# sarpel/wakeword_trainer_home

Hardware: AMD Instinct MI355X
Metric: training samples/sec (16kHz x 1.5s clips) (higher is better)
Workload: dtype bf16; 1 GPU; BASELINE config 2: cnn_small + log-mel(40) + SpecAugment, fwd/bwd + clip + AdamW, 16 kHz x 1.5 s clips resident in HBM; batch_per_gpu=512, activation_storage=bf16, arithmetic=f32, global_batch=512, n_samples=24000, parallelism=single, ranks_seen=1, hip_graph=False

## Files before the change

### include/wwhip.h

```cpp
#ifndef WWHIP_H
#define WWHIP_H

#include <stddef.h>
#include <stdint.h>

#ifdef __cplusplus
extern "C" {
#endif

#define WW_ABI_VERSION 15

#define WW_OK 0
#define WW_E_INVALID (-1)
#define WW_E_HIP (-2)
#define WW_E_WORKSPACE (-3)
#define WW_E_UNSUPPORTED (-4)

typedef struct ww_ctx ww_ctx;
typedef void *ww_stream_t;

int ww_abi_version(void);
const char *ww_last_error(void);
int ww_ctx_create(int device, ww_ctx **out);
int ww_ctx_destroy(ww_ctx *ctx);

typedef struct {
    uint64_t step;
    float lr;
    int32_t parity;
    float loss_scale;
    int32_t growth_tracker;
    int32_t reserved[2];
} ww_step_ctl;
int ww_ctx_bind_step_ctl(ww_ctx *ctx, const ww_step_ctl *ctl_dev );
int ww_step_ctl_advance(ww_ctx *ctx, ww_stream_t stream);

typedef struct {
    int32_t sample_rate;
    int32_t n_fft;
    int32_t hop;
    int32_t n_mels;
    int32_t n_mfcc;
    float f_min;
// ... 44 lines not shown
                     uint64_t sample_offset, int32_t *choice_out, void *scratch, size_t scratch_bytes,
                     ww_stream_t stream);

typedef struct {
    const float *gamma;
    const float *beta;
    float *running_mean;
    float *running_var;
    float momentum;
    float eps;
    int32_t training;
} ww_bn_t;

#define WW_C 64
#define WW_ACT_F32 0
#define WW_ACT_BF16 1
#define WW_ACT_F16 2
#define WW_MAX_PARTIALS 1024
size_t ww_layer_scratch_bytes(void);

int ww_conv_stem_fwd(ww_ctx *ctx, int act_dtype, const float *x, const float *w, int B, int Hin, int Win, void *y,
                     const ww_bn_t *bn, float *ss_out, float *mr_out, void *scratch, ww_stream_t stream);
int ww_dwconv3x3_fwd(ww_ctx *ctx, int act_dtype, const void *y_in, const float *ss_in, const float *w, int B, int H,
                     int W, void *y, const ww_bn_t *bn, float *ss_out, float *mr_out, void *scratch,
                     ww_stream_t stream);
int ww_pwconv1x1_fwd(ww_ctx *ctx, int act_dtype, const void *y_in, const float *ss_in, const float *w, int B, int H,
                     int W, void *y, const ww_bn_t *bn, float *ss_out, float *mr_out, void *scratch,
                     ww_stream_t stream);
int ww_gap_fwd(ww_ctx *ctx, int act_dtype, const void *y, const float *ss, const float *mr, int B, int H, int W,
               float *pool, ww_stream_t stream);
int ww_head_fwd(ww_ctx *ctx, const float *pool, int B, int HW, const float *fc_w, const float *fc_b,
                float dropout_p, int training, uint64_t seed, uint64_t step, uint64_t sample_offset, float *pd,
                float *logits, ww_stream_t stream);

int ww_head_bwd(ww_ctx *ctx, const float *dlogits, const float *pd, const float *pool, int B, int HW,
                const float *fc_w, float dropout_p, int training, uint64_t seed, uint64_t step,
                uint64_t sample_offset, const float *gamma_last, const float *mr_last, float *dfc_w,
                float *dfc_b, float *dpool, float *coef_last, float *dgamma_last, float *dbeta_last,
                ww_stream_t stream);
int ww_pwconv1x1_bwd(ww_ctx *ctx, int act_dtype, const void *g, const float *dpool, const void *y_out,
                     const float *ss_out, const float *coef, const void *y_in, const float *ss_in, const float *mr_in,
                     const float *gamma_in, const float *w, int B, int H, int W, void *g_in, float *dw,
                     float *coef_in, float *dgamma_in, float *dbeta_in, void *scratch, ww_stream_t stream);
int ww_dwconv3x3_bwd(ww_ctx *ctx, int act_dtype, const void *g, const void *y_out, const float *coef, const void *y_in,
                     const float *ss_in, const float *mr_in, const float *gamma_in, const float *w, int B,
                     int H, int W, void *g_in, float *dw, float *coef_in, float *dgamma_in,
                     float *dbeta_in, void *scratch, ww_stream_t stream);
int ww_conv_stem_bwd(ww_ctx *ctx, int act_dtype, const void *g, const void *y_out, const float *coef, const float *x,
                     int B, int Hin, int Win, float *dw, void *scratch, ww_stream_t stream);

#define WW_CNN_SMALL_NPTR 47
size_t ww_cnn_small_workspace_bytes(int B, int F, int T, int act_dtype);
int ww_cnn_small_fwd(ww_ctx *ctx, int act_dtype, void *const *params, const float *x, int B, int F, int T, int training,
                     float bn_momentum, float bn_eps, float dropout_p, uint64_t seed, uint64_t step,
                     uint64_t sample_offset, void *ws, size_t ws_bytes, float *logits, ww_stream_t stream);
#define WW_BWD_ALL 0
#define WW_BWD_LATE 1
#define WW_BWD_EARLY 2
int ww_cnn_small_bwd(ww_ctx *ctx, int act_dtype, void *const *params, void *const *grads, const float *x, const float *dlogits,
                     int B, int F, int T, float dropout_p, uint64_t seed, uint64_t step, uint64_t sample_offset,
                     void *ws, size_t ws_bytes, int part, ww_stream_t stream);

#define WW_LOSS_CE 0
#define WW_LOSS_FOCAL 1
typedef struct {
    float loss;
// ... 155 lines not shown
```

### wakeword_trainer_home_amd/_native.py

```python
import contextlib
import ctypes as C
import math
import os
from pathlib import Path

import torch

_LIB_PATH = Path(__file__).resolve().parent / "csrc" / "libwwhip.so"
_lib = None
_ctx = {}

ABI_VERSION = 15
BWD_ALL, BWD_LATE, BWD_EARLY = 0, 1, 2
ACT_F32, ACT_BF16, ACT_F16 = 0, 1, 2
LOSS_CE, LOSS_FOCAL = 0, 1
WAVE_F32, WAVE_I16 = 0, 1
CNN_SMALL_NPTR = 47


class NativeError(RuntimeError):
    pass


class FeatCfg(C.Structure):
    _fields_ = [("sample_rate", C.c_int32), ("n_fft", C.c_int32), ("hop", C.c_int32), ("n_mels", C.c_int32),
                ("n_mfcc", C.c_int32), ("f_min", C.c_float), ("f_max", C.c_float), ("log_eps", C.c_float)]


class SpecAugCfg(C.Structure):
    _fields_ = [("freq_mask_param", C.c_int32), ("time_mask_param", C.c_int32), ("n_freq_masks", C.c_int32),
                ("n_time_masks", C.c_int32), ("freq_mask_prob", C.c_float), ("time_mask_prob", C.c_float)]


class BN(C.Structure):
    _fields_ = [("gamma", C.c_void_p), ("beta", C.c_void_p), ("running_mean", C.c_void_p),
                ("running_var", C.c_void_p), ("momentum", C.c_float), ("eps", C.c_float), ("training", C.c_int32)]


class AudioAugCfg(C.Structure):
    _fields_ = [("rir_prob", C.c_float), ("noise_prob", C.c_float), ("snr_min_db", C.c_float), ("snr_max_db", C.c_float)]


class LinearEpi(C.Structure):
    _fields_ = [("act", C.c_int32), ("dropout_p", C.c_float), ("seed", C.c_uint64), ("step", C.c_uint64),
                ("sample_offset", C.c_uint64)]
# ... 89 lines not shown
    "ww_dwconv_nhwc_fwd": (C.c_int, [_vp, _vp, _vp, _i, _i, _i, _i, _i, _i, _vp, _vp]),
    "ww_dwconv_nhwc_bwd": (C.c_int, [_vp, _vp, _vp, _vp, _i, _i, _i, _i, _i, _i, _vp, _vp, _vp, _vp]),
    "ww_pool_hw_fwd": (C.c_int, [_vp, _vp, _i, _i, _i, _vp, _vp]),
    "ww_scale_bc_fwd": (C.c_int, [_vp, _vp, _vp, _i, _i, _i, _vp, _vp]),
    "ww_scale_bc_bwd_gate": (C.c_int, [_vp, _vp, _vp, _i, _i, _i, _vp, _vp]),
    "ww_scale_pool_bwd": (C.c_int, [_vp, _vp, _vp, _vp, _i, _i, _i, _vp, _vp]),
    "ww_se_bwd_scratch_bytes": (_sz, [_i, _i, _i]),
    "ww_se_fwd": (C.c_int, [_vp, _vp, _i, _i, _i, _i] + [_vp] * 9),
    "ww_se_bwd": (C.c_int, [_vp] * 8 + [_i, _i, _i, _i] + [_vp] * 6 + [_sz, _vp]),
    "ww_stem3x3s2_bn_act_fwd": (C.c_int, [_vp, _vp, _vp, _i, _i, _i, _i, C.POINTER(BN), _i, _vp, _vp, _vp, _vp, _vp, _vp]),
    "ww_stem3x3s2_bwd_dw": (C.c_int, [_vp, _vp, _vp, _i, _i, _i, _i, _vp, _vp, _vp]),
    "ww_im2col3x3s2": (C.c_int, [_vp, _vp, _i, _i, _i, _vp, _vp]),
    "ww_add_f32": (C.c_int, [_vp, _vp, _vp, _sz, _vp, _vp]),
    "ww_gru_workspace_bytes": (_sz, [_i, _i, _i, _i]),
    "ww_gru_fwd": (C.c_int, [_vp, _i, _vp, C.c_long, _vp, _vp, _vp, _vp, _vp, _i, _i, _i, _i, _i, _vp, C.c_long, _vp, _vp, _sz, _vp]),
    "ww_gru_bidir_fwd": (C.c_int, [_vp, _i, _vp, C.c_long, _vp, _i, _i, _i, _i, _vp, C.c_long, _sz, _vp]),
    "ww_gru_bidir_bwd": (C.c_int, [_vp, _i, _vp, C.c_long, _vp, _vp, C.c_long, _i, _i, _i, _i, _sz, _vp, C.c_long, _vp]),
    "ww_gru_bwd": (C.c_int, [_vp, _i, _vp, C.c_long, _vp, _vp, _vp, C.c_long, _vp, _i, _i, _i, _i, _i, _vp, _sz, _vp, C.c_long, _i,
                             _vp, _vp, _vp, _vp, _vp, _vp]),
    "ww_lstm_workspace_bytes": (_sz, [_i, _i, _i, _i]),
    "ww_lstm_fwd": (C.c_int, [_vp, _i, _vp, C.c_long, _vp, _vp, _vp, _vp, _vp, _vp, _i, _i, _i, _i, _i, _vp, C.c_long, _vp, _vp, _vp,
                              _sz, _vp]),
    "ww_lstm_bwd": (C.c_int, [_vp, _i, _vp, C.c_long, _vp, _vp, _vp, C.c_long, _vp, _vp, _i, _i, _i, _i, _i, _vp, _sz, _vp, C.c_long,
                              _i, _vp, _vp, _vp, _vp, _vp, _vp, _vp]),
    "ww_lstm_bidir_fwd": (C.c_int, [_vp, _i, _vp, C.c_long, _vp, _i, _i, _i, _i, _vp, C.c_long, _sz, _vp]),
    "ww_lstm_bidir_bwd": (C.c_int, [_vp, _i, _vp, C.c_long, _vp, _vp, C.c_long, _i, _i, _i, _i, _sz, _vp, C.c_long, _vp]),
    "ww_clip_optim_step": (C.c_int, [_vp, C.POINTER(OptimCfg), _vp, _vp, _vp, _vp, _sz, _vp, _i, _vp, _vp, _vp, _vp, _vp, _vp, _vp]),
    "ww_layer_scratch_bytes": (_sz, []),
    "ww_conv_stem_fwd": (C.c_int, [_vp, _i, _vp, _vp, _i, _i, _i, _vp, C.POINTER(BN), _vp, _vp, _vp, _vp]),
    "ww_dwconv3x3_fwd": (C.c_int, [_vp, _i, _vp, _vp, _vp, _i, _i, _i, _vp, C.POINTER(BN), _vp, _vp, _vp, _vp]),
    "ww_pwconv1x1_fwd": (C.c_int, [_vp, _i, _vp, _vp, _vp, _i, _i, _i, _vp, C.POINTER(BN), _vp, _vp, _vp, _vp]),
    "ww_gap_fwd": (C.c_int, [_vp, _i, _vp, _vp, _vp, _i, _i, _i, _vp, _vp]),
    "ww_head_fwd": (C.c_int, [_vp, _vp, _i, _i, _vp, _vp, _f, _i, _u64, _u64, _u64, _vp, _vp, _vp]),
    "ww_head_bwd": (C.c_int, [_vp, _vp, _vp, _vp, _i, _i, _vp, _f, _i, _u64, _u64, _u64, _vp, _vp, _vp, _vp, _vp, _vp,
                              _vp, _vp, _vp]),
    "ww_pwconv1x1_bwd": (C.c_int, [_vp, _i] + [_vp] * 10 + [_i, _i, _i] + [_vp] * 7),
    "ww_dwconv3x3_bwd": (C.c_int, [_vp, _i] + [_vp] * 8 + [_i, _i, _i] + [_vp] * 7),
    "ww_conv_stem_bwd": (C.c_int, [_vp, _i, _vp, _vp, _vp, _vp, _i, _i, _i, _vp, _vp, _vp]),
    "ww_cnn_small_workspace_bytes": (_sz, [_i, _i, _i, _i]),
    "ww_cnn_small_fwd": (C.c_int, [_vp, _i, C.POINTER(_vp), _vp, _i, _i, _i, _i, _f, _f, _f, _u64, _u64, _u64, _vp, _sz,
                                   _vp, _vp]),
    "ww_cnn_front_fwd": (C.c_int, [_vp, _i, C.POINTER(_vp), _vp, _i, _i, _i, _i, _f, _f, _vp, _sz, _vp, _vp]),
    "ww_cnn_front_bwd": (C.c_int, [_vp, _i, C.POINTER(_vp), C.POINTER(_vp), _vp, _vp, _i, _i, _i, _vp, _sz, _vp]),
    "ww_cnn_small_bwd": (C.c_int, [_vp, _i, C.POINTER(_vp), C.POINTER(_vp), _vp, _vp, _i, _i, _i, _f, _u64, _u64, _u64,
                                   _vp, _sz, _i, _vp]),
    "ww_ce2_loss_fwd_bwd": (C.c_int, [_vp, _vp, _vp, _i, _i, _f, _f, _f, _vp, _vp, _vp, _vp, _vp, _i, _vp]),
    "ww_grad_norm_clip": (C.c_int, [_vp, _vp, _sz, _f, _vp, _vp, _vp]),
    "ww_prof_num_classes": (C.c_int, []),
    "ww_prof_class_name": (C.c_char_p, [_i]),
    "ww_ctx_set_deferred_reduce": (C.c_int, [_vp, _i]),
    "ww_deferred_reduce_pending": (C.c_int, [_vp]),
    "ww_deferred_reduce_flush": (C.c_int, [_vp, _vp]),
    "ww_deferred_reduce_discard": (C.c_int, [_vp]),
    "ww_prof_enable": (C.c_int, [_vp, C.c_uint32]),
    "ww_prof_collect": (C.c_int, [_vp, C.POINTER(C.c_float), C.POINTER(C.c_int32)]),
    "ww_prob_threshold": (_u64, [C.c_double]),
    "ww_philox4x32_10": (None, [C.POINTER(C.c_uint32), C.POINTER(C.c_uint32), C.POINTER(C.c_uint32)]),
}
EXPORTS = tuple(_SIGS)


def lib_path() -> Path:
    return _LIB_PATH


def load():
# ... 821 lines not shown
                                     _p(scratch), _stream(dev)), name)
    return y, ss, mr


def dwconv3x3_fwd(y_in, ss_in, w, bn, scratch):
    return _conv_fwd("ww_dwconv3x3_fwd", y_in, ss_in, w, bn, scratch)


def pwconv1x1_fwd(y_in, ss_in, w, bn, scratch):
    return _conv_fwd("ww_pwconv1x1_fwd", y_in, ss_in, w, bn, scratch)


def gap_fwd(y, ss, mr):
    dev = _dev(y, ss, mr)
    B, H, W, _ = y.shape
    pool = torch.empty((B, 3, 64), dtype=torch.float32, device=dev)
    with _guard(dev):
        _check(load().ww_gap_fwd(ctx(dev), act_code(y.dtype), _p(y), _p(ss), _p(mr), B, H, W, _p(pool), _stream(dev)),
               "ww_gap_fwd")
    return pool


def head_fwd(pool, HW, fc_w, fc_b, dropout_p=0.0, training=True, seed=0, step=0, sample_offset=0):
    dev = _dev(pool, fc_w, fc_b)
    B = pool.shape[0]
    pd = torch.empty((B, 64), dtype=torch.float32, device=dev)
    logits = torch.empty((B, 2), dtype=torch.float32, device=dev)
    with _guard(dev):
        _check(load().ww_head_fwd(ctx(dev), _p(pool), B, HW, _p(fc_w), _p(fc_b), dropout_p, int(training), seed, step,
                                  sample_offset, _p(pd), _p(logits), _stream(dev)), "ww_head_fwd")
    return pd, logits


def head_bwd(dlogits, pd, pool, HW, fc_w, gamma_last, mr_last, dropout_p=0.0, training=True, seed=0, step=0,
             sample_offset=0):
    dev = _dev(dlogits, pd, pool, fc_w, gamma_last, mr_last)
    B = pool.shape[0]
    f32 = dict(dtype=torch.float32, device=dev)
    dfc_w, dfc_b = torch.empty((2, 64), **f32), torch.empty(2, **f32)
    dpool, coef = torch.empty((B, 64), **f32), torch.empty(192, **f32)
    dgamma, dbeta = torch.empty(64, **f32), torch.empty(64, **f32)
    with _guard(dev):
        _check(load().ww_head_bwd(ctx(dev), _p(dlogits), _p(pd), _p(pool), B, HW, _p(fc_w), dropout_p, int(training),
                                  seed, step, sample_offset, _p(gamma_last), _p(mr_last), _p(dfc_w), _p(dfc_b),
                                  _p(dpool), _p(coef), _p(dgamma), _p(dbeta), _stream(dev)), "ww_head_bwd")
    return dfc_w, dfc_b, dpool, coef, dgamma, dbeta


def pwconv1x1_bwd(g, dpool, y_out, ss_out, coef, y_in, ss_in, mr_in, gamma_in, w, scratch):
    dev = _dev(g, dpool, y_out, ss_out, coef, y_in, ss_in, mr_in, gamma_in, w, scratch)
    B, H, W, _ = y_out.shape
    f32 = dict(dtype=torch.float32, device=dev)
    g_in, dw = torch.empty_like(y_in), torch.empty((64, 64), **f32)
    coef_in, dgamma, dbeta = torch.empty(192, **f32), torch.empty(64, **f32), torch.empty(64, **f32)
    with _guard(dev):
        _check(load().ww_pwconv1x1_bwd(ctx(dev), act_code(y_out.dtype), _p(g), _p(dpool), _p(y_out), _p(ss_out), _p(coef), _p(y_in), _p(ss_in),
                                       _p(mr_in), _p(gamma_in), _p(w), B, H, W, _p(g_in), _p(dw), _p(coef_in),
                                       _p(dgamma), _p(dbeta), _p(scratch), _stream(dev)), "ww_pwconv1x1_bwd")
    return g_in, dw, coef_in, dgamma, dbeta


def dwconv3x3_bwd(g, y_out, coef, y_in, ss_in, mr_in, gamma_in, w, scratch):
    dev = _dev(g, y_out, coef, y_in, ss_in, mr_in, gamma_in, w, scratch)
    B, H, W, _ = y_out.shape
    f32 = dict(dtype=torch.float32, device=dev)
    g_in, dw = torch.empty_like(y_in), torch.empty((64, 1, 3, 3), **f32)
# ... 124 lines not shown
```

### wakeword_trainer_home_amd/csrc/ww_conv_bwd.hip

```cpp
#include "ww_internal.h"
#include <stdlib.h>
#include "ww_act.h"

namespace {

typedef float floatx16 __attribute__((ext_vector_type(16)));

constexpr int PW_LD = 68;


__global__ __launch_bounds__(1024) void k_head_bwd(const float *__restrict__ dlogits, const float *__restrict__ pd,
                                                  const float *__restrict__ pool, int B, int HW,
                                                  const float *__restrict__ fc_w, float drop_scale,
                                                  uint64_t drop_thresh, int use_dropout, uint32_t seed_lo,
                                                  uint32_t seed_hi, uint32_t step_lo, uint32_t step_hi,
                                                  uint64_t sample_offset, const float *__restrict__ gamma,
                                                  const float *__restrict__ mr, float *__restrict__ dfc_w,
                                                  float *__restrict__ dfc_b, float *__restrict__ dpool,
                                                  float *__restrict__ coef, float *__restrict__ dgamma,
                                                  float *__restrict__ dbeta, const ww_step_ctl *__restrict__ ctl) {
    __shared__ double sh[6][1024];
    __shared__ double sh2[6][16][8];
    ww_step_resolve(ctl, step_lo, step_hi, step_lo, step_hi);
    const int c = 8 * blockIdx.x + (threadIdx.x & 7), part = threadIdx.x >> 3;
// ... 555 lines not shown
#pragma unroll
    for (int t = 0; t < 9; ++t) {
        sh[slot * 576 + (2 * cl) * 9 + t] = dwa[t];
        sh[slot * 576 + (2 * cl + 1) * 9 + t] = dwb[t];
    }
    __syncthreads();
    for (int i = tid; i < 576; i += 256) {
        float t = 0.f;
#pragma unroll
        for (int s = 0; s < 8; ++s) t += sh[s * 576 + i];
        dw_partials[(size_t)blockIdx.x * 576 + i] = t;
    }
}

template <typename T, bool RECOMP>
__global__ __launch_bounds__(256) void k_stem_bwd(const T *__restrict__ g, const T *__restrict__ y_out,
                                                  const float *__restrict__ w, const float *__restrict__ coef,
                                                  const float *__restrict__ x, int B, int Hin, int Win, int Ho, int Wo,
                                                  float *__restrict__ dw_partials, int rev) {
    __shared__ float sh[8 * 576];
    extern __shared__ float xs[];
    const int tid = threadIdx.x, slot = tid >> 5, cl = tid & 31;
    const int ld = Win + 2;
    const float2 cA = *reinterpret_cast<const float2 *>(coef + 2 * cl);
    const float2 cB = *reinterpret_cast<const float2 *>(coef + 64 + 2 * cl);
    const float2 cC = *reinterpret_cast<const float2 *>(coef + 128 + 2 * cl);
    float dwa[9], dwb[9], w0[9], w1[9];
#pragma unroll
    for (int t = 0; t < 9; ++t) {
        dwa[t] = dwb[t] = 0.f;
        w0[t] = RECOMP ? w[(2 * cl) * 9 + t] : 0.f;
        w1[t] = RECOMP ? w[(2 * cl + 1) * 9 + t] : 0.f;
    }
    const long nrows = (long)B * Ho;
    float pre[2];
    auto fetch = [&](long item) {
        if (rev) item = nrows - 1 - item;
        const int fb_ = (int)(item / Ho), foh = (int)(item - (long)fb_ * Ho);
        const float *xb = x + (size_t)fb_ * Hin * Win;
#pragma unroll
        for (int k = 0; k < 2; ++k) {
            const int i = tid + 256 * k;
            const int kh = i / ld, c = i - kh * ld;
            const int ih = 2 * foh - 1 + kh, iw = c - 1;
            pre[k] = (i < 3 * ld && ih >= 0 && ih < Hin && iw >= 0 && iw < Win) ? xb[(size_t)ih * Win + iw] : 0.f;
        }
    };
    const bool ahead = 3 * ld <= 2 * 256;
    if (ahead && (long)blockIdx.x < nrows) fetch(blockIdx.x);
    for (long rowi = blockIdx.x; rowi < nrows; rowi += gridDim.x) {
        const long row = rev ? nrows - 1 - rowi : rowi;
        const int b = (int)(row / Ho), oh = (int)(row - (long)b * Ho);
        __syncthreads();
        if (ahead) {
#pragma unroll
            for (int k = 0; k < 2; ++k)
                if (tid + 256 * k < 3 * ld) xs[tid + 256 * k] = pre[k];
        } else {
            const float *xb = x + (size_t)b * Hin * Win;
            for (int i = tid; i < 3 * ld; i += 256) {
                const int kh = i / ld, c = i - kh * ld;
                const int ih = 2 * oh - 1 + kh, iw = c - 1;
                xs[i] = (ih >= 0 && ih < Hin && iw >= 0 && iw < Win) ? xb[(size_t)ih * Win + iw] : 0.f;
            }
        }
        __syncthreads();
        if (ahead && rowi + gridDim.x < nrows) fetch(rowi + gridDim.x);
        for (int ow0 = slot; ow0 < Wo; ow0 += 80) {
            typename Act<T>::raw2 gr[10], yr[10];
#pragma unroll
            for (int j = 0; j < 10; ++j) {
                const int ow = min(ow0 + 8 * j, Wo - 1);
                const size_t o = ((size_t)row * Wo + ow) * 64 + 2 * cl;
                gr[j] = Act<T>::ldraw2_nt(g + o);
                if constexpr (!RECOMP) yr[j] = Act<T>::ldraw2(y_out + o);
            }
#pragma unroll
            for (int j = 0; j < 10; ++j) {
                const int ow = ow0 + 8 * j;
                if (ow < Wo) {
                    const float2 gz = Act<T>::cvt2(gr[j]);
                    float v[9];
#pragma unroll
                    for (int kh = 0; kh < 3; ++kh)
#pragma unroll
                        for (int kw = 0; kw < 3; ++kw) v[kh * 3 + kw] = xs[kh * ld + 2 * ow + kw];
                    float2 yo;
                    if constexpr (RECOMP) {
                        float a0 = 0.f, a1 = 0.f;
#pragma unroll
                        for (int t = 0; t < 9; ++t) {
                            a0 = fmaf(v[t], w0[t], a0);
                            a1 = fmaf(v[t], w1[t], a1);
                        }
                        yo = Act<T>::round2(make_float2(a0, a1));
                    } else {
                        yo = Act<T>::cvt2(yr[j]);
                    }
                    const float d0 = fmaf(cA.x, gz.x, fmaf(cB.x, yo.x, cC.x));
                    const float d1 = fmaf(cA.y, gz.y, fmaf(cB.y, yo.y, cC.y));
#pragma unroll
                    for (int t = 0; t < 9; ++t) {
                        dwa[t] = fmaf(d0, v[t], dwa[t]);
                        dwb[t] = fmaf(d1, v[t], dwb[t]);
                    }
                }
            }
        }
// ... 207 lines not shown
```

### wakeword_trainer_home_amd/csrc/ww_conv_fwd.hip

```cpp
#include "ww_internal.h"
#include "ww_act.h"

namespace {

typedef float floatx16 __attribute__((ext_vector_type(16)));

__device__ __forceinline__ float bnrelu(float y, float s, float t) {
    const float z = fmaf(y, s, t);
    return z < 0.f ? 0.f : z;
}

__device__ __forceinline__ void reduce_stats_slots(float s0, float s1, float q0, float q1, float *sh ,
                                                   float *__restrict__ partial_row) {
    const int tid = threadIdx.x, slot = tid >> 5, cl = tid & 31;
    __syncthreads();
    sh[slot * 128 + 2 * cl] = s0;
    sh[slot * 128 + 2 * cl + 1] = s1;
    sh[slot * 128 + 64 + 2 * cl] = q0;
    sh[slot * 128 + 64 + 2 * cl + 1] = q1;
    __syncthreads();
    if (tid < 128) {
        float t = 0.f;
#pragma unroll
        for (int s = 0; s < 8; ++s) t += sh[s * 128 + tid];
// ... 367 lines not shown
                const int prow = rbase + (reg & 3) + 8 * (reg >> 2) + 4 * h;
                const float v = A16::round1(acc[reg]);
                otile[prow * PWH_LD + 32 * n + r] = (H)v;
                s1 += v;
                s2 = fmaf(v, v, s2);
            }
        }
        __syncthreads();
#pragma unroll
        for (int i = 0; i < 8; ++i) {
            const int row = (tid >> 4) + 16 * i;
            if (p0 + row < M)
                *reinterpret_cast<uint2 *>(y + (size_t)(p0 + row) * 64 + 4 * c4) =
                    *reinterpret_cast<const uint2 *>(otile + row * PWH_LD + 4 * c4);
        }
    }
    if (partials) {
        s1 += __shfl_xor(s1, 32);
        s2 += __shfl_xor(s2, 32);
        __syncthreads();
        float *sh = reinterpret_cast<float *>(otile);
        if (h == 0) {
            sh[wv * 64 + r] = s1;
            sh[wv * 64 + 32 + r] = s2;
        }
        __syncthreads();
        if (tid < 128) {
            const int kind = tid >> 6, c = tid & 63, nn = c >> 5, rr = c & 31;
            partials[(size_t)blockIdx.x * 128 + tid] = sh[nn * 64 + kind * 32 + rr] + sh[(2 + nn) * 64 + kind * 32 + rr];
        }
    }
}

template <typename T>
__global__ __launch_bounds__(1024) void k_gap_fwd(const T *__restrict__ y, const float *__restrict__ ss,
                                                  const float *__restrict__ mr, int HW, float *__restrict__ pool) {
    __shared__ __align__(16) float sh[64 * 192];
    const int tid = threadIdx.x, slot = tid >> 4, cl = tid & 15, b = blockIdx.x;
    const float4 sc = *reinterpret_cast<const float4 *>(ss + 4 * cl);
    const float4 sf = *reinterpret_cast<const float4 *>(ss + 64 + 4 * cl);
    const float4 mu = *reinterpret_cast<const float4 *>(mr + 4 * cl);
    const float4 rs = *reinterpret_cast<const float4 *>(mr + 64 + 4 * cl);
    const T *yb = y + (size_t)b * HW * 64 + 4 * cl;
    float4 a = make_float4(0.f, 0.f, 0.f, 0.f), h = a, c = a;
    auto one = [](float v, float scv, float sfv, float muv, float rsv, float &av, float &hv, float &cv) {
        const float z = fmaf(v, scv, sfv);
        av += z < 0.f ? 0.f : z;
        if (z > 0.f) { hv += (v - muv) * rsv; cv += 1.f; }
    };
    for (int p0 = slot; p0 < HW; p0 += 8 * 64) {
        typename Act<T>::raw4 r[8];
#pragma unroll
        for (int u = 0; u < 8; ++u) r[u] = Act<T>::ldraw4_nt(yb + (size_t)min(p0 + 64 * u, HW - 1) * 64);
#pragma unroll
        for (int u = 0; u < 8; ++u)
            if (p0 + 64 * u < HW) {
                const float4 v = Act<T>::cvt4(r[u]);
                one(v.x, sc.x, sf.x, mu.x, rs.x, a.x, h.x, c.x);
                one(v.y, sc.y, sf.y, mu.y, rs.y, a.y, h.y, c.y);
                one(v.z, sc.z, sf.z, mu.z, rs.z, a.z, h.z, c.z);
                one(v.w, sc.w, sf.w, mu.w, rs.w, a.w, h.w, c.w);
            }
    }
    *reinterpret_cast<float4 *>(sh + slot * 192 + 4 * cl) = a;
    *reinterpret_cast<float4 *>(sh + slot * 192 + 64 + 4 * cl) = h;
    *reinterpret_cast<float4 *>(sh + slot * 192 + 128 + 4 * cl) = c;
    __syncthreads();
    if (tid < 192) {
        float t = 0.f;
#pragma unroll 8
        for (int s = 0; s < 64; ++s) t += sh[s * 192 + tid];
        pool[(size_t)b * 192 + tid] = t;
    }
}

__global__ __launch_bounds__(256) void k_head_fwd(const float *__restrict__ pool, int B, int HW,
                                                  const float *__restrict__ fc_w, const float *__restrict__ fc_b,
                                                  float drop_scale, uint64_t drop_thresh, int use_dropout,
                                                  uint32_t seed_lo, uint32_t seed_hi, uint32_t step_lo, uint32_t step_hi,
                                                  uint64_t sample_offset, float *__restrict__ pd,
                                                  float *__restrict__ logits, const ww_step_ctl *__restrict__ ctl) {
    const int lane = threadIdx.x & 63, b = blockIdx.x * 4 + (threadIdx.x >> 6);
    if (b >= B) return;
    ww_step_resolve(ctl, step_lo, step_hi, step_lo, step_hi);
    float v = pool[(size_t)b * 192 + lane] / (float)HW;
    if (use_dropout) {
        uint32_t rr[4];
        ww_philox(step_lo, step_hi, (uint32_t)(sample_offset + (uint64_t)b), (WW_TAG_DROPOUT << 24) | (uint32_t)(lane >> 2),
                  seed_lo, seed_hi, rr);
        const uint32_t d = rr[lane & 3];
        v = ((uint64_t)d >= drop_thresh) ? v * drop_scale : 0.f;
    }
    pd[(size_t)b * 64 + lane] = v;
    float l0 = v * fc_w[lane], l1 = v * fc_w[64 + lane];
#pragma unroll
    for (int o = 32; o > 0; o >>= 1) {
        l0 += __shfl_xor(l0, o);
        l1 += __shfl_xor(l1, o);
    }
    if (lane == 0) {
        logits[(size_t)b * 2] = l0 + fc_b[0];
        logits[(size_t)b * 2 + 1] = l1 + fc_b[1];
    }
}

// ... 111 lines not shown
    g.B = B; g.H = H; g.W = W;
    g.ncs = (W + 3) / 4;
    g.nseg = (H + DW_HS - 1) / DW_HS;
    g.hs_len = (H + g.nseg - 1) / g.nseg;
    g.items = (long)B * g.nseg * g.ncs;
    hipStream_t st = (hipStream_t)stream;
    float *partials = bn->training ? (float *)scratch : nullptr;
    int grid = 0;
    rc = act_dtype == WW_ACT_BF16  ? launch_dw_fwd<ww_bf16>(ctx, y_in, ss_in, w, g, y, partials, &grid, st)
         : act_dtype == WW_ACT_F16 ? launch_dw_fwd<ww_f16>(ctx, y_in, ss_in, w, g, y, partials, &grid, st)
                                   : launch_dw_fwd<float>(ctx, y_in, ss_in, w, g, y, partials, &grid, st);
    if (rc) return rc;
    return finish_bn(ctx, partials, grid, (double)B * H * W, bn, ss_out, mr_out, st);
}

extern "C" int ww_pwconv1x1_fwd(ww_ctx *ctx, int act_dtype, const void *y_in, const float *ss_in, const float *w,
                                int B, int H, int W, void *y, const ww_bn_t *bn, float *ss_out, float *mr_out,
                                void *scratch, ww_stream_t stream) {
    WW_REQUIRE(ctx && y_in && ss_in && w && y, WW_E_INVALID, "ww_pwconv1x1_fwd: null argument");
    WW_REQUIRE(B >= 1 && H >= 1 && W >= 1, WW_E_INVALID, "ww_pwconv1x1_fwd: bad shape (%d,%d,%d)", B, H, W);
    int rc = check_bn("ww_pwconv1x1_fwd", bn, ss_out, mr_out, scratch);
    if (rc || (rc = check_act("ww_pwconv1x1_fwd", act_dtype))) return rc;
    const long M = (long)B * H * W;
    hipStream_t st = (hipStream_t)stream;
    float *partials = bn->training ? (float *)scratch : nullptr;
    int grid = 0;
    rc = act_dtype == WW_ACT_BF16  ? launch_pw_fwd_bf16<ww_bf16>(ctx, y_in, ss_in, w, M, y, partials, &grid, st)
         : act_dtype == WW_ACT_F16 ? launch_pw_fwd_bf16<ww_f16>(ctx, y_in, ss_in, w, M, y, partials, &grid, st)
                                   : launch_pw_fwd<float>(ctx, y_in, ss_in, w, M, y, partials, &grid, st);
    if (rc) return rc;
    return finish_bn(ctx, partials, grid, (double)M, bn, ss_out, mr_out, st);
}

extern "C" int ww_gap_fwd(ww_ctx *ctx, int act_dtype, const void *y, const float *ss, const float *mr, int B, int H,
                          int W, float *pool, ww_stream_t stream) {
    WW_REQUIRE(ctx && y && ss && mr && pool, WW_E_INVALID, "ww_gap_fwd: null argument");
    WW_REQUIRE(B >= 1 && H >= 1 && W >= 1, WW_E_INVALID, "ww_gap_fwd: bad shape (%d,%d,%d)", B, H, W);
    int rc = check_act("ww_gap_fwd", act_dtype);
    if (rc) return rc;
    hipStream_t st = (hipStream_t)stream;
    {
        ww_prof_scope ps_(ctx, WW_K_GAP_FWD, st);
        if (act_dtype == WW_ACT_BF16)
            hipLaunchKernelGGL(k_gap_fwd<ww_bf16>, dim3(B), dim3(1024), 0, st, (const ww_bf16 *)y, ss, mr, H * W, pool);
        else if (act_dtype == WW_ACT_F16)
            hipLaunchKernelGGL(k_gap_fwd<ww_f16>, dim3(B), dim3(1024), 0, st, (const ww_f16 *)y, ss, mr, H * W, pool);
        else
            hipLaunchKernelGGL(k_gap_fwd<float>, dim3(B), dim3(1024), 0, st, (const float *)y, ss, mr, H * W, pool);
    }
    WW_LAUNCH_CHECK();
    return WW_OK;
}

extern "C" int ww_head_fwd(ww_ctx *ctx, const float *pool, int B, int HW, const float *fc_w, const float *fc_b,
                           float dropout_p, int training, uint64_t seed, uint64_t step, uint64_t sample_offset,
                           float *pd, float *logits, ww_stream_t stream) {
    WW_REQUIRE(ctx && pool && fc_w && fc_b && pd && logits, WW_E_INVALID, "ww_head_fwd: null argument");
    WW_REQUIRE(B >= 1 && HW >= 1, WW_E_INVALID, "ww_head_fwd: bad shape (%d,%d)", B, HW);
    WW_REQUIRE(dropout_p >= 0.f && dropout_p < 1.f, WW_E_INVALID, "ww_head_fwd: dropout_p=%f not in [0,1)", dropout_p);
    const int use_dropout = training && dropout_p > 0.f;
    const float scale = (float)(1.0 / (1.0 - (double)dropout_p));
    ww_prof_scope ps_(ctx, WW_K_HEAD_LOSS, (hipStream_t)stream);
    hipLaunchKernelGGL(k_head_fwd, dim3((B + 3) / 4), dim3(256), 0, (hipStream_t)stream, pool, B, HW, fc_w, fc_b,
                       scale, ww_prob_threshold((double)dropout_p), use_dropout, (uint32_t)seed, (uint32_t)(seed >> 32),
                       (uint32_t)step, (uint32_t)(step >> 32), sample_offset, pd, logits, ctx->step_ctl);
    WW_LAUNCH_CHECK();
    return WW_OK;
}
```

### wakeword_trainer_home_amd/csrc/ww_model.hip

```cpp
#include "ww_internal.h"
#include "ww_act.h"
#include <algorithm>

namespace {

constexpr int NL = 9;

struct Layout {
    int Ho, Wo;
    size_t A;
    size_t y[NL], g[2], ss[NL], mr[NL], coef[NL], pool, pd, dpool, scratch, total;
};

Layout make_layout(int B, int F, int T, int act_dtype) {
    Layout L;
    L.Ho = (F + 1) / 2;
    L.Wo = (T + 1) / 2;
    L.A = (size_t)B * L.Ho * L.Wo * 64;
    const size_t esz = act_dtype == WW_ACT_F32 ? 4 : 2;
    size_t o = 0;
    auto takeb = [&](size_t bytes) { size_t r = o; o += (bytes + 255) & ~(size_t)255; return r; };
    auto take = [&](size_t nfloat) { return takeb(nfloat * sizeof(float)); };
    for (int i = 0; i < NL; ++i) L.y[i] = takeb(L.A * esz);
    L.g[0] = takeb(L.A * esz);
// ... 141 lines not shown
            s2a = fmaf(gv.x, (v.x - mu.x) * rs.x, s2a);
            s2b = fmaf(gv.y, (v.y - mu.y) * rs.y, s2b);
        }
    }
    sh[grp * 128 + 2 * cl] = s1a;       sh[grp * 128 + 2 * cl + 1] = s1b;
    sh[grp * 128 + 64 + 2 * cl] = s2a;  sh[grp * 128 + 64 + 2 * cl + 1] = s2b;
    __syncthreads();
    if (threadIdx.x < 128) {
        float t = 0.f;
#pragma unroll
        for (int q = 0; q < 8; ++q) t += sh[q * 128 + threadIdx.x];
        stat_partials[(size_t)blockIdx.x * 128 + threadIdx.x] = t;
    }
}

}

extern "C" size_t ww_cnn_small_workspace_bytes(int B, int F, int T, int act_dtype) {
    if (B < 1 || F < 1 || T < 1) return 0;
    return make_layout(B, F, T, act_dtype).total;
}

extern "C" int ww_cnn_small_fwd(ww_ctx *ctx, int act_dtype, void *const *params, const float *x, int B, int F, int T, int training,
                                float bn_momentum, float bn_eps, float dropout_p, uint64_t seed, uint64_t step,
                                uint64_t sample_offset, void *ws, size_t ws_bytes, float *logits, ww_stream_t stream) {
    int rc = check_common("ww_cnn_small_fwd", ctx, act_dtype, params, x, B, F, T, ws, ws_bytes);
    if (rc) return rc;
    WW_REQUIRE(logits != nullptr, WW_E_INVALID, "ww_cnn_small_fwd: logits is null");
    const Layout L = make_layout(B, F, T, act_dtype);
    char *w = (char *)ws;
    auto Fp = [&](size_t off) { return (float *)(w + off); };
    rc = conv_stack_fwd(ctx, act_dtype, params, x, B, F, T, training, bn_momentum, bn_eps, L, w, stream);
    if (rc) return rc;
    rc = ww_gap_fwd(ctx, act_dtype, w + L.y[8], Fp(L.ss[8]), Fp(L.mr[8]), B, L.Ho, L.Wo, Fp(L.pool), stream);
    if (rc) return rc;
    return ww_head_fwd(ctx, Fp(L.pool), B, L.Ho * L.Wo, (const float *)params[45], (const float *)params[46], dropout_p,
                       training, seed, step, sample_offset, Fp(L.pd), logits, stream);
}

extern "C" int ww_cnn_small_bwd(ww_ctx *ctx, int act_dtype, void *const *params, void *const *grads, const float *x,
                                const float *dlogits, int B, int F, int T, float dropout_p, uint64_t seed, uint64_t step,
                                uint64_t sample_offset, void *ws, size_t ws_bytes, int part, ww_stream_t stream) {
    int rc = check_common("ww_cnn_small_bwd", ctx, act_dtype, params, x, B, F, T, ws, ws_bytes);
    if (rc) return rc;
    WW_REQUIRE(grads && dlogits, WW_E_INVALID, "ww_cnn_small_bwd: null argument");
    WW_REQUIRE(part == WW_BWD_ALL || part == WW_BWD_LATE || part == WW_BWD_EARLY, WW_E_INVALID,
               "ww_cnn_small_bwd: unknown part %d", part);
    const Layout L = make_layout(B, F, T, act_dtype);
    char *w = (char *)ws;
    auto Fp = [&](size_t off) { return (float *)(w + off); };
    auto G = [&](int i) { return (float *)grads[i]; };
    for (int l = 0; l < NL; ++l) {
        WW_REQUIRE(grads[widx(l)] && grads[bnidx(l)] && grads[bnidx(l) + 1], WW_E_INVALID,
                   "ww_cnn_small_bwd: missing gradient buffer for conv layer %d", l);
    }
    WW_REQUIRE(grads[45] && grads[46], WW_E_INVALID, "ww_cnn_small_bwd: missing classifier gradient buffers");
    const int HW = L.Ho * L.Wo;
    if (part != WW_BWD_EARLY) {
        rc = ww_head_bwd(ctx, dlogits, Fp(L.pd), Fp(L.pool), B, HW, (const float *)params[45], dropout_p, 1, seed, step,
                         sample_offset, (const float *)params[bnidx(8)], Fp(L.mr[8]), G(45), G(46), Fp(L.dpool),
                         Fp(L.coef[8]), G(bnidx(8)), G(bnidx(8) + 1), stream);
        if (rc) return rc;
    }
    return conv_stack_bwd(ctx, act_dtype, params, grads, x, B, F, T, L, w, true, stream, part);
}

extern "C" int ww_cnn_front_fwd(ww_ctx *ctx, int act_dtype, void *const *params, const float *x, int B, int F, int T, int training,
                                float bn_momentum, float bn_eps, void *ws, size_t ws_bytes, float *seq, ww_stream_t stream) {
    int rc = check_common("ww_cnn_front_fwd", ctx, act_dtype, params, x, B, F, T, ws, ws_bytes, 45);
    if (rc) return rc;
// ... 52 lines not shown
```

Measured before the change: 418,000 samples/s.

## Fuse GAP with classifier head and prefetch grads in stem backward

Adds a fused global-average-pool plus FC head forward kernel, so the forward pass issues one launch instead of two and drops the separate head kernel. The pooled value is divided by HW, dropped out with the same Philox stream, and reduced across a 64-lane wavefront. Separately, the stem/conv backward kernel now software-prefetches the next tile's gradient (and, for half types, output) loads into registers one iteration ahead, with asm barriers to keep constants in VGPRs. Both changes add register pressure in exchange for hiding load latency and removing a launch.

```diff
diff --git a/include/wwhip.h b/include/wwhip.h
--- a/include/wwhip.h
+++ b/include/wwhip.h
@@ -8,7 +8,7 @@
 extern "C" {
 #endif
 
-#define WW_ABI_VERSION 15
+#define WW_ABI_VERSION 16
 
 #define WW_OK 0
 #define WW_E_INVALID (-1)
@@ -119,6 +119,9 @@
 int ww_head_fwd(ww_ctx *ctx, const float *pool, int B, int HW, const float *fc_w, const float *fc_b,
                 float dropout_p, int training, uint64_t seed, uint64_t step, uint64_t sample_offset, float *pd,
                 float *logits, ww_stream_t stream);
+int ww_gap_head_fwd(ww_ctx *ctx, int act_dtype, const void *y, const float *ss, const float *mr, int B, int H, int W,
+                    const float *fc_w, const float *fc_b, float dropout_p, int training, uint64_t seed, uint64_t step,
+                    uint64_t sample_offset, float *pool, float *pd, float *logits, ww_stream_t stream);
 
 int ww_head_bwd(ww_ctx *ctx, const float *dlogits, const float *pd, const float *pool, int B, int HW,
                 const float *fc_w, float dropout_p, int training, uint64_t seed, uint64_t step,
diff --git a/wakeword_trainer_home_amd/_native.py b/wakeword_trainer_home_amd/_native.py
--- a/wakeword_trainer_home_amd/_native.py
+++ b/wakeword_trainer_home_amd/_native.py
@@ -10,7 +10,7 @@
 _lib = None
 _ctx = {}
 
-ABI_VERSION = 15
+ABI_VERSION = 16
 BWD_ALL, BWD_LATE, BWD_EARLY = 0, 1, 2
 ACT_F32, ACT_BF16, ACT_F16 = 0, 1, 2
 LOSS_CE, LOSS_FOCAL = 0, 1
@@ -166,6 +166,7 @@
     "ww_pwconv1x1_fwd": (C.c_int, [_vp, _i, _vp, _vp, _vp, _i, _i, _i, _vp, C.POINTER(BN), _vp, _vp, _vp, _vp]),
     "ww_gap_fwd": (C.c_int, [_vp, _i, _vp, _vp, _vp, _i, _i, _i, _vp, _vp]),
     "ww_head_fwd": (C.c_int, [_vp, _vp, _i, _i, _vp, _vp, _f, _i, _u64, _u64, _u64, _vp, _vp, _vp]),
+    "ww_gap_head_fwd": (C.c_int, [_vp, _i, _vp, _vp, _vp, _i, _i, _i, _vp, _vp, _f, _i, _u64, _u64, _u64, _vp, _vp, _vp, _vp]),
     "ww_head_bwd": (C.c_int, [_vp, _vp, _vp, _vp, _i, _i, _vp, _f, _i, _u64, _u64, _u64, _vp, _vp, _vp, _vp, _vp, _vp,
                               _vp, _vp, _vp]),
     "ww_pwconv1x1_bwd": (C.c_int, [_vp, _i] + [_vp] * 10 + [_i, _i, _i] + [_vp] * 7),
@@ -1053,6 +1054,19 @@
     return pd, logits
 
 
+def gap_head_fwd(y, ss, mr, fc_w, fc_b, dropout_p=0.0, training=True, seed=0, step=0, sample_offset=0):
+    dev = _dev(y, ss, mr, fc_w, fc_b)
+    B, H, W, _ = y.shape
+    pool = torch.empty((B, 3, 64), dtype=torch.float32, device=dev)
+    pd = torch.empty((B, 64), dtype=torch.float32, device=dev)
+    logits = torch.empty((B, 2), dtype=torch.float32, device=dev)
+    with _guard(dev):
+        _check(load().ww_gap_head_fwd(ctx(dev), act_code(y.dtype), _p(y), _p(ss), _p(mr), B, H, W, _p(fc_w), _p(fc_b),
+                                      dropout_p, int(training), seed, step, sample_offset, _p(pool), _p(pd), _p(logits),
+                                      _stream(dev)), "ww_gap_head_fwd")
+    return pool, pd, logits
+
+
 def head_bwd(dlogits, pd, pool, HW, fc_w, gamma_last, mr_last, dropout_p=0.0, training=True, seed=0, step=0,
              sample_offset=0):
     dev = _dev(dlogits, pd, pool, fc_w, gamma_last, mr_last)
diff --git a/wakeword_trainer_home_amd/csrc/ww_conv_bwd.hip b/wakeword_trainer_home_amd/csrc/ww_conv_bwd.hip
--- a/wakeword_trainer_home_amd/csrc/ww_conv_bwd.hip
+++ b/wakeword_trainer_home_amd/csrc/ww_conv_bwd.hip
@@ -611,6 +611,11 @@
         w0[t] = RECOMP ? w[(2 * cl) * 9 + t] : 0.f;
         w1[t] = RECOMP ? w[(2 * cl + 1) * 9 + t] : 0.f;
     }
+    asm volatile("" ::"v"(cA.x), "v"(cA.y), "v"(cB.x), "v"(cB.y), "v"(cC.x), "v"(cC.y));
+    if constexpr (RECOMP) {
+#pragma unroll
+        for (int t = 0; t < 9; ++t) asm volatile("" ::"v"(w0[t]), "v"(w1[t]));
+    }
     const long nrows = (long)B * Ho;
     float pre[2];
     auto fetch = [&](long item) {
@@ -625,8 +630,20 @@
             pre[k] = (i < 3 * ld && ih >= 0 && ih < Hin && iw >= 0 && iw < Win) ? xb[(size_t)ih * Win + iw] : 0.f;
         }
     };
+    constexpr bool Y_AHEAD = !RECOMP && !Act<T>::is_f32, Y_INTRIP = !RECOMP && Act<T>::is_f32;
+    typename Act<T>::raw2 gn[10] = {}, yn[10] = {};
+    auto gfetch = [&](long frow, int ow0) {
+        const size_t rb = (size_t)frow * Wo * 64;
+#pragma unroll
+        for (int j = 0; j < 10; ++j) {
+            const uint32_t o = (uint32_t)(ow0 < 0 ? 0 : min(ow0 + 8 * j, Wo - 1)) * 64 + 2 * cl;
+            gn[j] = Act<T>::ldraw2_nt(g + rb + o);
+            if constexpr (Y_AHEAD) yn[j] = Act<T>::ldraw2(y_out + rb + o);
+        }
+    };
     const bool ahead = 3 * ld <= 2 * 256;
     if (ahead && (long)blockIdx.x < nrows) fetch(blockIdx.x);
+    if ((long)blockIdx.x < nrows && slot < Wo) gfetch(rev ? nrows - 1 - blockIdx.x : (long)blockIdx.x, slot);
     for (long rowi = blockIdx.x; rowi < nrows; rowi += gridDim.x) {
         const long row = rev ? nrows - 1 - rowi : rowi;
         const int b = (int)(row / Ho), oh = (int)(row - (long)b * Ho);
@@ -649,10 +666,15 @@
             typename Act<T>::raw2 gr[10], yr[10];
 #pragma unroll
             for (int j = 0; j < 10; ++j) {
-                const int ow = min(ow0 + 8 * j, Wo - 1);
-                const size_t o = ((size_t)row * Wo + ow) * 64 + 2 * cl;
-                gr[j] = Act<T>::ldraw2_nt(g + o);
-                if constexpr (!RECOMP) yr[j] = Act<T>::ldraw2(y_out + o);
+                gr[j] = gn[j];
+                if constexpr (Y_AHEAD) yr[j] = yn[j];
+                if constexpr (Y_INTRIP)
+                    yr[j] = Act<T>::ldraw2(y_out + ((size_t)row * Wo + min(ow0 + 8 * j, Wo - 1)) * 64 + 2 * cl);
+            }
+            {
+                const bool same = ow0 + 80 < Wo, last = !same && rowi + gridDim.x >= nrows;
+                const long nrowi = rowi + gridDim.x;
+                gfetch((same || last) ? row : (rev ? nrows - 1 - nrowi : nrowi), same ? ow0 + 80 : last ? -1 : slot);
             }
 #pragma unroll
             for (int j = 0; j < 10; ++j) {
diff --git a/wakeword_trainer_home_amd/csrc/ww_conv_fwd.hip b/wakeword_trainer_home_amd/csrc/ww_conv_fwd.hip
--- a/wakeword_trainer_home_amd/csrc/ww_conv_fwd.hip
+++ b/wakeword_trainer_home_amd/csrc/ww_conv_fwd.hip
@@ -423,9 +423,21 @@
     }
 }
 
-template <typename T>
+struct GapHead {
+    const float *fc_w, *fc_b;
+    float drop_scale;
+    uint64_t drop_thresh;
+    int use_dropout;
+    uint32_t seed_lo, seed_hi, step_lo, step_hi;
+    uint64_t sample_offset;
+    float *pd, *logits;
+    const ww_step_ctl *ctl;
+};
+
+template <typename T, bool HEAD>
 __global__ __launch_bounds__(1024) void k_gap_fwd(const T *__restrict__ y, const float *__restrict__ ss,
-                                                  const float *__restrict__ mr, int HW, float *__restrict__ pool) {
+                                                  const float *__restrict__ mr, int HW, float *__restrict__ pool,
+                                                  GapHead hd) {
     __shared__ __align__(16) float sh[64 * 192];
     const int tid = threadIdx.x, slot = tid >> 4, cl = tid & 15, b = blockIdx.x;
     const float4 sc = *reinterpret_cast<const float4 *>(ss + 4 * cl);
@@ -462,6 +474,32 @@
 #pragma unroll 8
         for (int s = 0; s < 64; ++s) t += sh[s * 192 + tid];
         pool[(size_t)b * 192 + tid] = t;
+        if constexpr (HEAD) {
+            if (tid < 64) {
+                const int lane = tid;
+                uint32_t step_lo, step_hi;
+                ww_step_resolve(hd.ctl, hd.step_lo, hd.step_hi, step_lo, step_hi);
+                float v = t / (float)HW;
+                if (hd.use_dropout) {
+                    uint32_t rr[4];
+                    ww_philox(step_lo, step_hi, (uint32_t)(hd.sample_offset + (uint64_t)b),
+                              (WW_TAG_DROPOUT << 24) | (uint32_t)(lane >> 2), hd.seed_lo, hd.seed_hi, rr);
+                    const uint32_t d = rr[lane & 3];
+                    v = ((uint64_t)d >= hd.drop_thresh) ? v * hd.drop_scale : 0.f;
+                }
+                hd.pd[(size_t)b * 64 + lane] = v;
+                float l0 = v * hd.fc_w[lane], l1 = v * hd.fc_w[64 + lane];
+#pragma unroll
+                for (int o = 32; o > 0; o >>= 1) {
+                    l0 += __shfl_xor(l0, o);
+                    l1 += __shfl_xor(l1, o);
+                }
+                if (lane == 0) {
+                    hd.logits[(size_t)b * 2] = l0 + hd.fc_b[0];
+                    hd.logits[(size_t)b * 2 + 1] = l1 + hd.fc_b[1];
+                }
+            }
+        }
     }
 }
 
@@ -639,24 +677,55 @@
     return finish_bn(ctx, partials, grid, (double)M, bn, ss_out, mr_out, st);
 }
 
+template <bool HEAD>
+int launch_gap(ww_ctx *ctx, int act_dtype, const void *y, const float *ss, const float *mr, int B, int HW, float *pool,
+               const GapHead &hd, hipStream_t st) {
+    {
+        ww_prof_scope ps_(ctx, WW_K_GAP_FWD, st);
+        if (act_dtype == WW_ACT_BF16)
+            hipLaunchKernelGGL((k_gap_fwd<ww_bf16, HEAD>), dim3(B), dim3(1024), 0, st, (const ww_bf16 *)y, ss, mr, HW, pool, hd);
+        else if (act_dtype == WW_ACT_F16)
+            hipLaunchKernelGGL((k_gap_fwd<ww_f16, HEAD>), dim3(B), dim3(1024), 0, st, (const ww_f16 *)y, ss, mr, HW, pool, hd);
+        else
+            hipLaunchKernelGGL((k_gap_fwd<float, HEAD>), dim3(B), dim3(1024), 0, st, (const float *)y, ss, mr, HW, pool, hd);
+    }
+    WW_LAUNCH_CHECK();
+    return WW_OK;
+}
+
 extern "C" int ww_gap_fwd(ww_ctx *ctx, int act_dtype, const void *y, const float *ss, const float *mr, int B, int H,
                           int W, float *pool, ww_stream_t stream) {
     WW_REQUIRE(ctx && y && ss && mr && pool, WW_E_INVALID, "ww_gap_fwd: null argument");
     WW_REQUIRE(B >= 1 && H >= 1 && W >= 1, WW_E_INVALID, "ww_gap_fwd: bad shape (%d,%d,%d)", B, H, W);
     int rc = check_act("ww_gap_fwd", act_dtype);
     if (rc) return rc;
-    hipStream_t st = (hipStream_t)stream;
-    {
-        ww_prof_scope ps_(ctx, WW_K_GAP_FWD, st);
-        if (act_dtype == WW_ACT_BF16)
-            hipLaunchKernelGGL(k_gap_fwd<ww_bf16>, dim3(B), dim3(1024), 0, st, (const ww_bf16 *)y, ss, mr, H * W, pool);
-        else if (act_dtype == WW_ACT_F16)
-            hipLaunchKernelGGL(k_gap_fwd<ww_f16>, dim3(B), dim3(1024), 0, st, (const ww_f16 *)y, ss, mr, H * W, pool);
-        else
-            hipLaunchKernelGGL(k_gap_fwd<float>, dim3(B), dim3(1024), 0, st, (const float *)y, ss, mr, H * W, pool);
-    }
-    WW_LAUNCH_CHECK();
-    return WW_OK;
+    return launch_gap<false>(ctx, act_dtype, y, ss, mr, B, H * W, pool, GapHead{}, (hipStream_t)stream);
+}
+
+extern "C" int ww_gap_head_fwd(ww_ctx *ctx, int act_dtype, const void *y, const float *ss, const float *mr, int B, int H,
+                               int W, const float *fc_w, const float *fc_b, float dropout_p, int training, uint64_t seed,
+                               uint64_t step, uint64_t sample_offset, float *pool, float *pd, float *logits,
+                               ww_stream_t stream) {
+    WW_REQUIRE(ctx && y && ss && mr && pool && fc_w && fc_b && pd && logits, WW_E_INVALID, "ww_gap_head_fwd: null argument");
+    WW_REQUIRE(B >= 1 && H >= 1 && W >= 1, WW_E_INVALID, "ww_gap_head_fwd: bad shape (%d,%d,%d)", B, H, W);
+    WW_REQUIRE(dropout_p >= 0.f && dropout_p < 1.f, WW_E_INVALID, "ww_gap_head_fwd: dropout_p=%f not in [0,1)", dropout_p);
+    int rc = check_act("ww_gap_head_fwd", act_dtype);
+    if (rc) return rc;
+    GapHead hd;
+    hd.fc_w = fc_w;
+    hd.fc_b = fc_b;
+    hd.drop_scale = (float)(1.0 / (1.0 - (double)dropout_p));
+    hd.drop_thresh = ww_prob_threshold((double)dropout_p);
+    hd.use_dropout = training && dropout_p > 0.f;
+    hd.seed_lo = (uint32_t)seed;
+    hd.seed_hi = (uint32_t)(seed >> 32);
+    hd.step_lo = (uint32_t)step;
+    hd.step_hi = (uint32_t)(step >> 32);
+    hd.sample_offset = sample_offset;
+    hd.pd = pd;
+    hd.logits = logits;
+    hd.ctl = ctx->step_ctl;
+    return launch_gap<true>(ctx, act_dtype, y, ss, mr, B, H * W, pool, hd, (hipStream_t)stream);
 }
 
 extern "C" int ww_head_fwd(ww_ctx *ctx, const float *pool, int B, int HW, const float *fc_w, const float *fc_b,
diff --git a/wakeword_trainer_home_amd/csrc/ww_model.hip b/wakeword_trainer_home_amd/csrc/ww_model.hip
--- a/wakeword_trainer_home_amd/csrc/ww_model.hip
+++ b/wakeword_trainer_home_amd/csrc/ww_model.hip
@@ -197,10 +197,9 @@
     auto Fp = [&](size_t off) { return (float *)(w + off); };
     rc = conv_stack_fwd(ctx, act_dtype, params, x, B, F, T, training, bn_momentum, bn_eps, L, w, stream);
     if (rc) return rc;
-    rc = ww_gap_fwd(ctx, act_dtype, w + L.y[8], Fp(L.ss[8]), Fp(L.mr[8]), B, L.Ho, L.Wo, Fp(L.pool), stream);
-    if (rc) return rc;
-    return ww_head_fwd(ctx, Fp(L.pool), B, L.Ho * L.Wo, (const float *)params[45], (const float *)params[46], dropout_p,
-                       training, seed, step, sample_offset, Fp(L.pd), logits, stream);
+    return ww_gap_head_fwd(ctx, act_dtype, w + L.y[8], Fp(L.ss[8]), Fp(L.mr[8]), B, L.Ho, L.Wo, (const float *)params[45],
+                           (const float *)params[46], dropout_p, training, seed, step, sample_offset, Fp(L.pool), Fp(L.pd),
+                           logits, stream);
 }
 
 extern "C" int ww_cnn_small_bwd(ww_ctx *ctx, int act_dtype, void *const *params, void *const *grads, const float *x,
```

Measured after the change: 419,200 samples/s (median of 6 runs). About the same (+0.3%).
